# OnurBasci/TransformerBasedNavierStokeSolver

Measured on AMD Instinct MI355X. Metric: ns64_train_samples_per_s, higher is better.
Workload: dtype f32

## Files before the change

transformerbasednavierstokesolver_amd/csrc/pa2d_gemm.hip:

```cpp
#include "pa2d_gemm_common.h"
#include <string.h>

static bool engine_ok(int e) { return e >= 0 && e <= 2; }

static Pa2dEnv read_env() {
    auto is = [](const char* n, const char* pre) { const char* e = getenv(n); return e && strncmp(e, pre, strlen(pre)) == 0; };
    auto num = [](const char* n, int dflt) { const char* e = getenv(n); return (e && e[0]) ? atoi(e) : dflt; };
    Pa2dEnv v;
    v.conv_halo = is("PA2D_CONV_HALO", "o") ? 0 : (is("PA2D_CONV_HALO", "f") ? 2 : 1);
    v.mc_big_off = is("PA2D_MC_BIG", "o") ? 1 : 0;
    v.kc_bk16 = num("PA2D_KC_BK", 0) == 16 ? 1 : 0;
    v.mc_bk = num("PA2D_MC_BK", 16) == 32 ? 32 : 16;
    v.mc_splits = num("PA2D_MC_SPLITS", 0);
    v.mcb_splits = num("PA2D_MCB_SPLITS", 0);
    v.lin_dw_split = is("PA2D_LIN_DW_SPLIT", "of") ? 0 : 1;
    v.lin_panel = is("PA2D_LIN_PANEL", "of") ? 0 : 1;
    v.lin_rowpanel = is("PA2D_LIN_ROWPANEL", "of") ? 0 : 1;
    v.lin_small_split = is("PA2D_LIN_SMALL_SPLIT", "of") ? 0 : 1;
    v.conv_mfma16 = num("PA2D_CONV_MFMA", 16) == 32 ? 0 : 1;
    v.split_big = num("PA2D_SPLIT_BIG", 1);
    v.slice_map = is("PA2D_SLICE_MAP", "l") ? 0 : 1;
    v.default_engine = is("PA2D_GEMM", "f") ? 0 : (is("PA2D_GEMM", "b") ? 2 : 1);
    return v;
}
static Pa2dEnv g_env = read_env();
const Pa2dEnv& pa2d_env() { return g_env; }
static int kc_bk(bool im2col, int Cin) {
    if (im2col && pa2d_env().kc_bk16) return 16;
    return (!im2col || (Cin % 32) == 0) ? 32 : 16;
}
KCTile kc_tile(int M, int N, bool im2col, int Cin) {
    const int tiles_m = ceil_div(M, 128);
    const long long t128 = (long long)tiles_m * ceil_div(N, 128);
    const long long t12864 = (long long)tiles_m * ceil_div(N, 64);
    const int bk = kc_bk(im2col, Cin);
    if (N > 64 && t128 >= 384) return {128, 128, bk};
    if (t12864 >= 384 || M <= 64) return {128, 64, bk};
    return {64, 64, bk};
}
bool use_split(int engine, int N, bool im2col, int Cin) {
    const int m = engine;
    if (m == 1) return im2col && N > 64 && (Cin % 32) == 0;
    if (m == 2) return N > 64 && (!im2col || (Cin % 32) == 0);
    return false;
}

static int launch_kc(const KCParams& p_in, bool im2col, hipStream_t st, hipEvent_t ev0 = nullptr, hipEvent_t ev1 = nullptr);
static int launch_kc(const KCParams& p_in, bool im2col, hipStream_t st, hipEvent_t ev0, hipEvent_t ev1) {
    KCParams p = p_in;
    if (!engine_ok(p.engine)) return PA2D_ERR_ARG;
    if (p.M <= 0 || p.N <= 0 || p.K <= 0) return PA2D_OK;
    if (!p.bias2) p.bias_split = 0x7fffffff;
    {
        const unsigned long long ab = ((unsigned long long)(p.M - 1) * p.lda + (im2col ? p.Cin : p.K)) * 4ull;
        const unsigned long long bb = ((unsigned long long)(p.N - 1) * p.ldb + p.K) * 4ull;
        if (ab >= 0xFFFFFFF0ull || bb >= 0xFFFFFFF0ull) return PA2D_ERR_UNSUPPORTED;
        p.a_bytes = (unsigned)ab;
        p.b_bytes = (unsigned)bb;
        const unsigned long long es = p.io_bf16 ? 2ull : 4ull;
        const unsigned long long cb = ((unsigned long long)(p.M - 1) * p.ldc + p.N) * es;
        const unsigned long long rb = p.res ? ((unsigned long long)(p.M - 1) * p.ldres + p.N) * es : 0ull;
        const unsigned long long xb = p.aux ? ((unsigned long long)(p.M - 1) * p.ldaux + p.N) * es : 0ull;
        if (cb >= 0xFFFFFFF0ull || rb >= 0xFFFFFFF0ull || xb >= 0xFFFFFFF0ull) return PA2D_ERR_UNSUPPORTED;
        p.c_bytes = (unsigned)cb; p.res_bytes = (unsigned)rb; p.aux_bytes = (unsigned)xb;
    }
    if ((p.K & 3) || (p.lda & 3) || (p.ldb & 3)) return PA2D_ERR_ARG;
    if (im2col && ((p.Cin & 15) || p.K != 9 * p.Cin)) return PA2D_ERR_UNSUPPORTED;
    if (im2col && (p.epi != 0 || p.res)) return PA2D_ERR_ARG;
    if (ev0 && hipEventRecord(ev0, st) != hipSuccess) return PA2D_ERR_ARG;
    int rc;
    if (!im2col && p.wimg && rowpanel_applies(p)) {
        if (p.wsrc) {
            rc = launch_pack_weight_image(p.wsrc, p.wsn, p.wsk, p.wimg, p.N, p.K, st);
            if (rc) return rc;
        }
        KCParams pp = p;
        pp.M = p.M - p.M % 128;
        rc = launch_kc_rowpanel(pp, p.wimg, st);
        if (!rc && pp.M < p.M) {
            KCParams pt = p_in;
            pt.wimg = nullptr;
            pt.M = p.M - pp.M;
            pt.A = p.A + (size_t)pp.M * p.lda;
            pt.C = p.C + (size_t)pp.M * p.ldc;
            if (p.res) pt.res = p.res + (size_t)pp.M * p.ldres;
            if (p.aux) pt.aux = p.aux + (size_t)pp.M * p.ldaux;
            rc = launch_kc(pt, false, st);
        }
    } else if (panel_applies(p, im2col)) {
        KCParams pp = p;
        pp.M = p.M - p.M % 256;
        rc = launch_kc_panel(pp, st);
        if (!rc && pp.M < p.M) {
            KCParams pt = p_in;
            const size_t ea = p.io_bf16 ? 2 : 4, es = p.io_bf16 ? 2 : 4;
            pt.M = p.M - pp.M;
            pt.A = (const float*)((const char*)p.A + (size_t)pp.M * p.lda * ea);
            pt.C = (float*)((char*)p.C + (size_t)pp.M * p.ldc * es);
            if (p.res) pt.res = (const float*)((const char*)p.res + (size_t)pp.M * p.ldres * es);
            if (p.aux) pt.aux = (float*)((char*)p.aux + (size_t)pp.M * p.ldaux * es);
            rc = launch_kc(pt, false, st);
        }
    } else if (p.io_bf16 || use_split(p.engine, p.N, im2col, p.Cin)) rc = launch_kc_split(p, im2col, st);
    else if (kc_split_small_applies(p, im2col)) rc = launch_kc_split_small(p, st);
    else rc = launch_kc_f32(p, im2col, kc_tile(p.M, p.N, im2col, p.Cin), st);
    if (rc) return rc;
    if (ev1 && hipEventRecord(ev1, st) != hipSuccess) return PA2D_ERR_ARG;
    return PA2D_OK;
}

__global__ void repack_kernel(const float* __restrict__ w0, const float* __restrict__ w1, float* __restrict__ dst,
                              int mode, int N, int K, int C, int Cin) {
    const long long idx = (long long)blockIdx.x * blockDim.x + threadIdx.x;
    if (mode == 0) {
        if (idx >= (long long)N * K) return;
        const int n = (int)(idx % N), k = (int)(idx / N);
        dst[idx] = w0[(size_t)n * K + k];
    } else if (mode == 1) {
        if (idx >= (long long)2 * C * 9 * Cin) return;
        const int CH = K;
        const int c16 = (int)(idx % CH);
        const int tap = (int)((idx / CH) % 9);
        const int cic = (int)((idx / (9 * CH)) % (Cin / CH));
        const int co = (int)(idx / ((long long)Cin * 9));
        const int ci = cic * CH + c16;
        const float* src = co < C ? w0 : w1;
        dst[idx] = src[((size_t)(co % C) * Cin + ci) * 9 + tap];
    } else {
        if (idx >= (long long)2 * C * 9 * Cin) return;
        const int CH = K;
        const int c16 = (int)(idx % CH);
        const int tap = (int)((idx / CH) % 9);
        const int cic = (int)((idx / (9 * CH)) % (2 * C / CH));
        const int ci = (int)(idx / ((long long)2 * C * 9));
        const int co = cic * CH + c16;
        const float* src = co < C ? w0 : w1;
        dst[idx] = src[((size_t)(co % C) * Cin + ci) * 9 + (8 - tap)];
    }
}

static int launch_repack(const float* w0, const float* w1, float* dst, int mode, int N, int K, int C, int Cin,
                         hipStream_t st) {
    const long long count = mode == 0 ? (long long)N * K : (long long)2 * C * 9 * Cin;
    hipLaunchKernelGGL(repack_kernel, dim3((unsigned)ceil_div_ll(count, 256)), dim3(256), 0, st, w0, w1, dst, mode,
                       N, K, C, Cin);
    PA2D_CHECK_LAUNCH();
    return PA2D_OK;
}

extern "C" {

int pa2d_default_engine(void) { return pa2d_env().default_engine; }

void pa2d_reload_env(void) { g_env = read_env(); }

size_t pa2d_gemm_fwd_workspace(int N, int K, int engine) { return rowpanel_image_bytes(N, K, engine); }
size_t pa2d_gemm_bwd_data_workspace(int N, int K, int engine) {
    return (size_t)N * K * sizeof(float) + rowpanel_image_bytes(K, N, engine);
}

int pa2d_gemm_weight_image(const float* w, long long ldw, int transposed, void* img, size_t img_bytes, int N, int K,
                           int engine, hipStream_t st) {
    const size_t need = rowpanel_image_bytes(N, K, engine);
    if (need == 0) return PA2D_ERR_UNSUPPORTED;
    if (!img || img_bytes < need) return PA2D_ERR_WORKSPACE;
    return transposed ? launch_pack_weight_image(w, 1, ldw, img, N, K, st) : launch_pack_weight_image(w, ldw, 1, img, N, K, st);
}

int pa2d_gemm_bias_act_fwd(const float* x, long long ldx, const float* w, long long ldw, const float* bias,
                           const float* res, long long ldres, float* y, long long ldy, float* pre, long long ldpre,
                           const void* wimg, void* ws, size_t ws_bytes, int M, int N, int K, int act, int engine,
                           hipStream_t st) {
    KCParams p = {};
    p.engine = engine;
    p.aux_deriv = (act & PA2D_ACT_SAVE_DERIVATIVE_BIT) ? 1 : 0;
    act &= ~PA2D_ACT_SAVE_DERIVATIVE_BIT;
    p.A = x; p.lda = ldx; p.B = w; p.ldb = ldw; p.C = y; p.ldc = ldy; p.bias = bias; p.res = res; p.ldres = ldres;
    p.aux = pre; p.ldaux = ldpre; p.M = M; p.N = N; p.K = K; p.act = act;
    p.epi = (act != ACT_NONE ? EPI_ACT : 0) | (pre ? EPI_STORE_PRE : 0);
    const size_t img = rowpanel_image_bytes(N, K, engine);
    if (img && wimg) p.wimg = const_cast<void*>(wimg);
    else if (ws && img && ws_bytes >= img) { p.wimg = ws; p.wsrc = w; p.wsn = ldw; p.wsk = 1; }
    return launch_kc(p, false, st);
}

int pa2d_gemm_bwd_data(const float* dy, long long lddy, const float* w, long long ldw, const float* pre,
                       long long ldpre, int act, float* dx, long long lddx, const void* wimg, void* ws, size_t ws_bytes, int M,
                       int N, int K, int engine, hipStream_t st) {
    if (ldw != K) return PA2D_ERR_ARG;
    if (N & 3) return PA2D_ERR_ARG;
    if (M <= 0) return PA2D_OK;
    if (ws_bytes < (size_t)N * K * sizeof(float)) return PA2D_ERR_WORKSPACE;
    float* const wt_ws = (float*)ws;
    KCParams p = {};
    p.engine = engine;
    p.aux_deriv = (act & PA2D_ACT_SAVE_DERIVATIVE_BIT) ? 1 : 0;
    act &= ~PA2D_ACT_SAVE_DERIVATIVE_BIT;
    p.A = dy; p.lda = lddy; p.B = wt_ws; p.ldb = N; p.C = dx; p.ldc = lddx; p.M = M; p.N = K; p.K = N;
    p.aux = const_cast<float*>(pre); p.ldaux = ldpre; p.act = act;
    p.epi = (pre && act != ACT_NONE) ? EPI_MUL_DACT : 0;
    const size_t img = rowpanel_image_bytes(K, N, engine);
    if (img && wimg) p.wimg = const_cast<void*>(wimg);
    else if (img && ws_bytes >= (size_t)N * K * sizeof(float) + img) {
        p.wimg = (char*)ws + (size_t)N * K * sizeof(float); p.wsrc = w; p.wsn = 1; p.wsk = ldw;
    }
    if (!(p.wimg && rowpanel_applies(p) && (M % 128) == 0)) {
        const int rc = launch_repack(w, nullptr, wt_ws, 0, N, K, 0, 0, st);
        if (rc) return rc;
    }
    return launch_kc(p, false, st);
}

size_t pa2d_gemm_bwd_weight_workspace(int M, int N, int K, int engine) {
    (void)engine;
    const MCPlan pl = plan_mc(N, K, M);
    return (pl.slab_floats + (size_t)pl.splits * N) * sizeof(float);
}

int pa2d_gemm_bwd_weight(const float* dy, long long lddy, const float* x, long long ldx, float* dw, float* db,
                         void* ws, size_t ws_bytes, int M, int N, int K, int accumulate, int engine, hipStream_t st) {
    if (!engine_ok(engine)) return PA2D_ERR_ARG;
    if (M <= 0) {
        if (accumulate) return PA2D_OK;
        const int rz = pa2d_zero(dw, sizeof(float) * N * K, st);
        return rz ? rz : pa2d_zero(db, sizeof(float) * N, st);
    }
    if (ws_bytes < pa2d_gemm_bwd_weight_workspace(M, N, K, engine)) return PA2D_ERR_WORKSPACE;
    const MCPlan pl = plan_mc(N, K, M);
    float* cs = db ? (float*)ws + pl.slab_floats : nullptr;
    const bool bfk = (engine == 1 || engine == 2) && pl.big && mc_f32src_applies(N, K, M, lddy, ldx);
    int rc = bfk ? launch_mc_f32src(dy, lddy, N, x, ldx, K, M, (float*)ws, pl, engine == 2 ? 1 : 3, cs, st)
                 : launch_mc(dy, lddy, N, x, ldx, K, M, false, 0, 0, 0, (float*)ws, pl, engine, st, cs);
    if (rc) return rc;
    rc = launch_reduce((const float*)ws, pl.splits, (long long)N * K, dw, nullptr, 0, 0, 0, st, accumulate);
    if (rc) return rc;
    if (db) rc = launch_reduce(cs, pl.splits, N, db, nullptr, 0, 0, 0, st, accumulate);
    return rc;
}

static size_t conv_planes_bytes(int engine, int M, int N, int Cin) {
    if (!use_split(engine, N, true, Cin)) return 0;
    return (planes_bytes(M, Cin, engine == 2 ? 1 : 3) + 255) & ~(size_t)255;
}

static int conv_dw_kind(int engine, int M, int C) {
    if (conv_planes_bytes(engine, M, C, 2 * C) == 0) return 0;
    if (mc_planes_big_applies(C, C, M)) return 2;
    return (mc_planes_supported(C, C) && plan_mc(2 * C, 9 * C, M).big) ? 1 : 0;
}
static MCPlan conv_dw_plan(int engine, int M, int C) {
    return conv_dw_kind(engine, M, C) == 2 ? plan_mc_planes_big(2 * C, 9 * C, M) : plan_mc(2 * C, 9 * C, M);
}
static size_t conv_xplanes_bytes(int engine, int M, int C) {
    return conv_dw_kind(engine, M, C) ? ((planes_bytes(M, C, engine == 2 ? 1 : 3) + 255) & ~(size_t)255) : 0;
}

size_t pa2d_conv3x3x2_workspace(int B, int H, int W, int C, int engine) {
    const size_t pack = (size_t)3 * C * 9 * C;
    const MCPlan pl = conv_dw_plan(engine, B * H * W, C);
    size_t sl = pl.slab_floats, cs = (size_t)colsum_blocks(B * H * W) * 2 * C;
    return (pack + (sl > cs ? sl : cs)) * sizeof(float) + conv_planes_bytes(engine, B * H * W, C, 2 * C) +
           conv_xplanes_bytes(engine, B * H * W, C);
}

size_t pa2d_conv3x3x2_fwd_workspace(int B, int H, int W, int C, int engine) {
    return (size_t)3 * C * 9 * C * sizeof(float) + conv_planes_bytes(engine, B * H * W, 2 * C, C);
}

static int conv_pack(const float* wx, const float* wf, float* pack, int M, int C, int direction, int engine,
                     hipStream_t st) {
    const int N = direction ? C : 2 * C, Cin = direction ? 2 * C : C;
    if (use_split(engine, N, true, Cin)) {
        return launch_repack_split(wx, wf, pack, direction, engine == 2 ? 1 : 3, C, C, st);
    }
    return launch_repack(wx, wf, pack, direction ? 2 : 1, 0, kc_tile(M, N, true, Cin).bk, C, C, st);
}

size_t pa2d_conv3x3x2_pack_bytes(int C) { return (size_t)3 * C * 9 * C * sizeof(float); }

int pa2d_conv3x3x2_pack(const float* wx, const float* wf, void* pack, size_t pack_bytes, int B, int H, int W, int C,
                        int direction, int engine, hipStream_t st) {
    if (!engine_ok(engine)) return PA2D_ERR_ARG;
    if (pack_bytes < pa2d_conv3x3x2_pack_bytes(C)) return PA2D_ERR_WORKSPACE;
    return conv_pack(wx, wf, (float*)pack, B * H * W, C, direction ? 1 : 0, engine, st);
}

int pa2d_conv3x3x2_fwd(const float* xn, const float* wx, const float* bx, const float* wf, const float* bf,
                       float* out, const void* prepacked, void* ws, size_t ws_bytes, int B, int H, int W, int C,
                       int engine, hipStream_t st, hipEvent_t ev_start, hipEvent_t ev_stop) {
    if (!engine_ok(engine)) return PA2D_ERR_ARG;
    if (B <= 0) return PA2D_OK;
    if (ws_bytes < pa2d_conv3x3x2_fwd_workspace(B, H, W, C, engine)) return PA2D_ERR_WORKSPACE;
    const float* pack = (const float*)prepacked;
    if (!pack) {
        const int rc = conv_pack(wx, wf, (float*)ws, B * H * W, C, 0, engine, st);
        if (rc) return rc;
        pack = (const float*)ws;
    }
    const size_t apl = conv_planes_bytes(engine, B * H * W, 2 * C, C);
    void* const planes = (char*)ws + pa2d_conv3x3x2_pack_bytes(C);
    if (apl) {
        const int rc = launch_split_planes(xn, C, planes, (long long)B * H * W, C, engine == 2 ? 1 : 3, st);
        if (rc) return rc;
    }
    KCParams p = {};
    p.engine = engine;
    p.A = apl ? (const float*)planes : xn; p.apre = apl ? 1 : 0;
    p.lda = C; p.B = pack; p.ldb = 9 * C; p.C = out; p.ldc = 2 * C;
    p.bias = bx; p.bias2 = bf; p.bias_split = C;
    p.M = B * H * W; p.N = 2 * C; p.K = 9 * C; p.H = H; p.W = W; p.Cin = C;
    return launch_kc(p, true, st, ev_start, ev_stop);
}

int pa2d_conv3x3x2_bwd(const float* dout, const float* xn, const float* wx, const float* wf, float* dxn, float* dwx,
                       float* dbx, float* dwf, float* dbf, const void* prepacked, void* ws, size_t ws_bytes, int B,
                       int H, int W, int C, int accumulate, int engine, hipStream_t st, hipEvent_t ev_start,
                       hipEvent_t ev_stop) {
    if (!engine_ok(engine)) return PA2D_ERR_ARG;
    if (B <= 0) {
        if (accumulate) return PA2D_OK;
        const size_t wb = sizeof(float) * (size_t)C * C * 9, bb = sizeof(float) * C;
        int rz = pa2d_zero(dwx, wb, st);
// ... 259 lines not shown
```

transformerbasednavierstokesolver_amd/csrc/pa2d_gemm_mc_planes.hip:

```cpp
#include "pa2d_gemm_common.h"

typedef short s16x4 __attribute__((ext_vector_type(4)));
typedef short s16x8 __attribute__((ext_vector_type(8)));

struct MCPlanesParams {
    const void* PA; int chA;
    const void* PB; int chB;
    float* slab;
    int Mi, Nj, Mk, chunks_per_split, splits, H, W, Cin;
    unsigned a_bytes, b_bytes;
    int taps;
    long long lda, ldb;
    float* colsum;
};

__device__ __forceinline__ unsigned img_off(int row, int ch) {
    return 256u * row + 16u * (ch ^ (((row & 3) << 2) | ((row >> 2) & 3)));
}

template <int NT, int KS, bool F32SRC = false>
__global__ __launch_bounds__(256, 2) void gemm_mc_planes_kernel(const MCPlanesParams p) {
    constexpr int PIMG = 4096;
    constexpr int STAGE = 2 * NT * KS * PIMG;
    constexpr int NP = 2 * NT * KS;
// ... 80 lines not shown
            rg[s] = s_isb[s] ? __builtin_amdgcn_raw_buffer_load_b128(rb_rsrc, ok_ ? rowb_ + s_goff[s] : OOB_OFF, 0, 0) \
                             : __builtin_amdgcn_raw_buffer_load_b128(ra_rsrc, ok_ ? rowb_ + s_goff[s] : OOB_OFF, 0, 0); \
        }                                                                                                 \
    }
#define MP_STORE(buf_)                                                                                    \
    if constexpr (F32SRC) {                                                                               \
        _Pragma("unroll") for (int ks = 0; ks < KS; ++ks) _Pragma("unroll") for (int op = 0; op < 2; ++op) { \
            const u32x4 u0_ = rg[ks * 4 + op * 2], u1_ = rg[ks * 4 + op * 2 + 1];                         \
            const float4 v0_ = make_float4(__uint_as_float(u0_.x), __uint_as_float(u0_.y), __uint_as_float(u0_.z), __uint_as_float(u0_.w)); \
            const float4 v1_ = make_float4(__uint_as_float(u1_.x), __uint_as_float(u1_.y), __uint_as_float(u1_.z), __uint_as_float(u1_.w)); \
            if (op == 0 && do_cs) {                                                                       \
                cs[0] += v0_.x; cs[1] += v0_.y; cs[2] += v0_.z; cs[3] += v0_.w;                           \
                cs[4] += v1_.x; cs[5] += v1_.y; cs[6] += v1_.z; cs[7] += v1_.w;                           \
            }                                                                                             \
            bf16x4 h0_, m0_, l0_, h1_, m1_, l1_;                                                          \
            split3(v0_, h0_, m0_, l0_);                                                                   \
            split3(v1_, h1_, m1_, l1_);                                                                   \
            unsigned char* d_ = smem + (buf_) * STAGE + flds;                                             \
            *reinterpret_cast<bf16x8*>(d_ + ((op * NT + 0) * KS + ks) * PIMG) = __builtin_shufflevector(h0_, h1_, 0, 1, 2, 3, 4, 5, 6, 7); \
            if (NT == 3) {                                                                                \
                *reinterpret_cast<bf16x8*>(d_ + ((op * NT + 1) * KS + ks) * PIMG) = __builtin_shufflevector(m0_, m1_, 0, 1, 2, 3, 4, 5, 6, 7); \
                *reinterpret_cast<bf16x8*>(d_ + ((op * NT + 2) * KS + ks) * PIMG) = __builtin_shufflevector(l0_, l1_, 0, 1, 2, 3, 4, 5, 6, 7); \
            }                                                                                             \
        }                                                                                                 \
    } else {                                                                                              \
        _Pragma("unroll") for (int s = 0; s < NP; ++s)                                                    \
            *reinterpret_cast<u32x4*>(smem + (buf_) * STAGE + s_lds[s]) = rg[s];                          \
    }
    const bool do_cs = F32SRC && p.colsum != nullptr && tj == 0;

    f32x16 acc[2][2];
#pragma unroll
    for (int i = 0; i < 2; ++i)
#pragma unroll
        for (int j = 0; j < 2; ++j)
#pragma unroll
            for (int r = 0; r < 16; ++r) acc[i][j][r] = 0.f;

    const int g = lane >> 4, q4 = (lane & 15) >> 2, pq = lane & 3;
    unsigned fa[2][2], fb[2][2];
#pragma unroll
    for (int t = 0; t < 2; ++t)
#pragma unroll
        for (int r = 0; r < 2; ++r) {
            const int row = 8 * (g >> 1) + 4 * r + q4;
            const int cha = ((wm * 64 + t * 32) >> 3) + 2 * (g & 1) + (pq >> 1);
            const int chb = ((wn * 64 + t * 32) >> 3) + 2 * (g & 1) + (pq >> 1);
            fa[t][r] = img_off(row, cha) + 8u * (pq & 1);
            fb[t][r] = img_off(row, chb) + 8u * (pq & 1);
        }

    if (c_begin < c_end) {
        MP_LOAD(c_begin)
        MP_STORE(0)
    }
    __syncthreads();
    for (int c = c_begin; c < c_end; c += KS) {
        const int buf = ((c - c_begin) / KS) & 1;
        if (c + KS < c_end) { MP_LOAD(c + KS) }
#pragma unroll
        for (int ks = 0; ks < KS; ++ks) {
        const unsigned char* st = smem + buf * STAGE + ks * PIMG;
        bf16x8 af[2][NT], bf[2][NT];
#pragma unroll
        for (int t = 0; t < 2; ++t)
#pragma unroll
            for (int pl = 0; pl < NT; ++pl) {
                typedef __attribute__((address_space(3))) s16x4 lds_s16x4;
                const s16x4 a0 = __builtin_amdgcn_ds_read_tr16_b64_v4i16((lds_s16x4*)(st + pl * KS * PIMG + fa[t][0]));
                const s16x4 a1 = __builtin_amdgcn_ds_read_tr16_b64_v4i16((lds_s16x4*)(st + pl * KS * PIMG + fa[t][1]));
                const s16x4 b0 = __builtin_amdgcn_ds_read_tr16_b64_v4i16((lds_s16x4*)(st + (NT + pl) * KS * PIMG + fb[t][0]));
                const s16x4 b1 = __builtin_amdgcn_ds_read_tr16_b64_v4i16((lds_s16x4*)(st + (NT + pl) * KS * PIMG + fb[t][1]));
                const s16x8 av = __builtin_shufflevector(a0, a1, 0, 1, 2, 3, 4, 5, 6, 7);
                const s16x8 bv = __builtin_shufflevector(b0, b1, 0, 1, 2, 3, 4, 5, 6, 7);
                af[t][pl] = __builtin_bit_cast(bf16x8, av);
                bf[t][pl] = __builtin_bit_cast(bf16x8, bv);
            }
#pragma unroll
        for (int i = 0; i < 2; ++i)
#pragma unroll
            for (int j = 0; j < 2; ++j) {
                if constexpr (NT == 3) {
                    acc[i][j] = __builtin_amdgcn_mfma_f32_32x32x16_bf16(af[i][1], bf[j][1], acc[i][j], 0, 0, 0);
                    acc[i][j] = __builtin_amdgcn_mfma_f32_32x32x16_bf16(af[i][2], bf[j][0], acc[i][j], 0, 0, 0);
                    acc[i][j] = __builtin_amdgcn_mfma_f32_32x32x16_bf16(af[i][0], bf[j][2], acc[i][j], 0, 0, 0);
                    acc[i][j] = __builtin_amdgcn_mfma_f32_32x32x16_bf16(af[i][1], bf[j][0], acc[i][j], 0, 0, 0);
                    acc[i][j] = __builtin_amdgcn_mfma_f32_32x32x16_bf16(af[i][0], bf[j][1], acc[i][j], 0, 0, 0);
                }
                acc[i][j] = __builtin_amdgcn_mfma_f32_32x32x16_bf16(af[i][0], bf[j][0], acc[i][j], 0, 0, 0);
            }
        }
        if (c + KS < c_end) { MP_STORE(buf ^ 1) }
        __syncthreads();
    }
#undef MP_LOAD
#undef MP_STORE

    if constexpr (F32SRC) {
        if (do_cs) {
            float* sm = reinterpret_cast<float*>(smem);
#pragma unroll
            for (int e = 0; e < 8; ++e) sm[frow * 128 + fc8 * 8 + e] = cs[e];
            __syncthreads();
            if (tid < 128) {
                float t = 0.f;
#pragma unroll
                for (int r = 0; r < 16; ++r) t += sm[r * 128 + tid];
                if (ti * 128 + tid < p.Mi) p.colsum[(size_t)split * p.Mi + ti * 128 + tid] = t;
            }
        }
    }
    float* out = p.slab + (size_t)split * p.Mi * p.Nj;
    const int col0 = tj * 128 + wn * 64 + (lane & 31);
    const int row0 = ti * 128 + wm * 64 + 4 * (lane >> 5);
#pragma unroll
    for (int j = 0; j < 2; ++j)
#pragma unroll
        for (int i = 0; i < 2; ++i)
#pragma unroll
            for (int r = 0; r < 16; ++r) {
                const int row = row0 + i * 32 + (r & 3) + 8 * (r >> 2);
                if (!F32SRC || (row < p.Mi && col0 + j * 32 < p.Nj)) out[(size_t)row * p.Nj + col0 + j * 32] = acc[i][j][r];
            }
}

bool mc_planes_supported(int C, int Cin) { return (C % 64) == 0 && (Cin % 128) == 0; }

int launch_mc_planes(const void* PA, const void* PB, int C, int Cin, int Mk, int H, int W, float* slab,
                     const MCPlan& pl, int NT, hipStream_t st) {
    if (!mc_planes_supported(C, Cin) || !pl.big) return PA2D_ERR_UNSUPPORTED;
    MCPlanesParams p;
    p.PA = PA; p.chA = 2 * C / 32; p.PB = PB; p.chB = Cin / 32; p.slab = slab;
    p.Mi = 2 * C; p.Nj = 9 * Cin; p.Mk = Mk; p.chunks_per_split = pl.chunks_per_split; p.splits = pl.splits;
    p.H = H; p.W = W; p.Cin = Cin; p.taps = 9;
    const unsigned long long ab = (unsigned long long)Mk * p.chA * NT * 64, bb = (unsigned long long)Mk * p.chB * NT * 64;
    if (ab >= 0xFFFFFFF0ull || bb >= 0xFFFFFFF0ull) return PA2D_ERR_UNSUPPORTED;
    p.a_bytes = (unsigned)ab; p.b_bytes = (unsigned)bb;
    const dim3 grid((p.Mi / 128) * (p.Nj / 128) * pl.splits);
    if (NT == 3) hipLaunchKernelGGL((gemm_mc_planes_kernel<3, 1>), grid, dim3(256), 0, st, p);
    else hipLaunchKernelGGL((gemm_mc_planes_kernel<1, 4>), grid, dim3(256), 0, st, p);
    PA2D_CHECK_LAUNCH();
    return PA2D_OK;
}

template <int NT, int KS>
__global__ __launch_bounds__(512, 1) void gemm_mc_planes_big_kernel(const MCPlanesParams p, const int per_xcd) {
    constexpr int PIMG = 8192;
    constexpr int STAGE = 2 * NT * KS * PIMG;
    constexpr int NP = (2 * NT * KS * 512) / 512;
    extern __shared__ __attribute__((aligned(16))) unsigned char smem[];

    const int tid = threadIdx.x, lane = tid & 63, wave = tid >> 6;
    const int tiles_i = (p.Mi + 255) / 256, tiles_j = (p.Nj + 255) / 256;
    const int tiles = tiles_i * tiles_j;
    const int lin = (blockIdx.x & 7) * per_xcd + (blockIdx.x >> 3);
    if ((int)(blockIdx.x >> 3) >= per_xcd || lin >= tiles * p.splits) return;
    const int split = lin / tiles, t_ = lin - split * tiles;
    const int ti = t_ / tiles_j, tj = t_ - ti * tiles_j;
    const int wm = wave >> 2, wn = wave & 3;
    const int total_chunks = (p.Mk + 15) / 16;
    const int c_begin = split * p.chunks_per_split;
    const int c_end = min(total_chunks, c_begin + p.chunks_per_split);
    const int HW = p.taps == 1 ? 1 : p.H * p.W;

    const __amdgpu_buffer_rsrc_t ra_rsrc = __builtin_amdgcn_make_buffer_rsrc(const_cast<void*>(p.PA), 0, p.a_bytes, 0x00020000);
    const __amdgpu_buffer_rsrc_t rb_rsrc = __builtin_amdgcn_make_buffer_rsrc(const_cast<void*>(p.PB), 0, p.b_bytes, 0x00020000);

    const int row16 = tid >> 5, cgrp = (tid & 31) >> 2, piece = tid & 3;
    const bool colok_a = ti * 256 + cgrp * 32 < p.Mi;
    const unsigned goff_a = (unsigned)((((ti * 256) >> 5) + cgrp) * NT * 64 + piece * 16);
    const int jc = tj * 256 + cgrp * 32;
    const int tap = p.taps == 1 ? 4 : jc / p.Cin;
    const bool colok_b = jc < p.Nj;
    const unsigned goff_b = (unsigned)((p.taps == 1 ? (jc >> 5) : ((jc - tap * p.Cin) >> 5)) * NT * 64 + piece * 16);
    const int tap_dy = tap / 3 - 1, tap_dx = tap - (tap / 3) * 3 - 1, tap_shift = tap_dy * p.W + tap_dx;
    const unsigned pitch_a = (unsigned)(p.chA * NT * 64), pitch_b = (unsigned)(p.chB * NT * 64);
    const unsigned lds_off = 512u * row16 + 16u * ((unsigned)(cgrp * 4 + piece) ^ (unsigned)(((row16 & 3) << 2) | ((row16 >> 2) & 3)));
#define MB_LOAD(c_, RG)                                                                                   \
    {                                                                                                     \
        _Pragma("unroll") for (int ks = 0; ks < KS; ++ks) {                                               \
            const int m_ = ((c_) + ks) * 16 + row16;                                                      \
            const bool okr_ = m_ < p.Mk && (c_) + ks < c_end;             \
            bool okb_ = okr_ && colok_b;                                                                  \
            int mm_ = m_;                                                                                 \
            if (p.taps != 1) {       \
                okb_ = okb_ && (unsigned)(ly + tap_dy) < (unsigned)p.H && (unsigned)(lx + tap_dx) < (unsigned)p.W; \
                mm_ = m_ + tap_shift;                                                                     \
                lx += 16;                                                                                 \
                while (lx >= p.W) { lx -= p.W; ++ly; }                                                    \
                while (ly >= p.H) ly -= p.H;                                                              \
            }                                                                                             \
            const unsigned oa_ = (okr_ && colok_a) ? (unsigned)m_ * pitch_a + goff_a : OOB_OFF;           \
            const unsigned ob_ = okb_ ? (unsigned)mm_ * pitch_b + goff_b : OOB_OFF;                       \
            _Pragma("unroll") for (int pl = 0; pl < NT; ++pl) {                                           \
                RG[pl * KS + ks] = __builtin_amdgcn_raw_buffer_load_b128(ra_rsrc, oa_ == OOB_OFF ? OOB_OFF : oa_ + pl * 64u, 0, 0); \
                RG[(NT + pl) * KS + ks] = __builtin_amdgcn_raw_buffer_load_b128(rb_rsrc, ob_ == OOB_OFF ? OOB_OFF : ob_ + pl * 64u, 0, 0); \
            }                                                                                             \
        }                                                                                                 \
    }
#define MB_STORE(buf_, RG)                                                                                \
    {                                                                                                     \
        _Pragma("unroll") for (int s = 0; s < NP; ++s)                                                    \
            *reinterpret_cast<u32x4*>(smem + (buf_) * STAGE + s * PIMG + lds_off) = RG[s];                \
    }
    u32x4 rg0[NP];
    int ly = 0, lx = 0;
    if (p.taps != 1) {
        const int n0 = (c_begin * 16 + row16) % HW;
        ly = n0 / p.W;
        lx = n0 - ly * p.W;
    }

    f32x16 acc[4][2];
#pragma unroll
    for (int i = 0; i < 4; ++i)
#pragma unroll
        for (int j = 0; j < 2; ++j)
#pragma unroll
            for (int r = 0; r < 16; ++r) acc[i][j][r] = 0.f;

    const int g = lane >> 4, q4 = (lane & 15) >> 2, pq = lane & 3;
    unsigned fa[4][2], fb[2][2];
#pragma unroll
    for (int r = 0; r < 2; ++r) {
        const int row = 8 * (g >> 1) + 4 * r + q4;
        const unsigned swz = (unsigned)(((row & 3) << 2) | ((row >> 2) & 3));
#pragma unroll
        for (int t = 0; t < 4; ++t) {
            const int cha = ((wm * 128 + t * 32) >> 3) + 2 * (g & 1) + (pq >> 1);
            fa[t][r] = 512u * row + 16u * ((unsigned)cha ^ swz) + 8u * (pq & 1);
        }
#pragma unroll
        for (int t = 0; t < 2; ++t) {
            const int chb = ((wn * 64 + t * 32) >> 3) + 2 * (g & 1) + (pq >> 1);
            fb[t][r] = 512u * row + 16u * ((unsigned)chb ^ swz) + 8u * (pq & 1);
        }
    }

#define MB_COMPUTE(buf_)                                                                                  \
    _Pragma("unroll") for (int ks = 0; ks < KS; ++ks) {                                                   \
        const unsigned char* st = smem + (buf_) * STAGE + ks * PIMG;                                      \
        bf16x8 af[4][NT], bf[2][NT];                                                                      \
        typedef __attribute__((address_space(3))) s16x4 lds_s16x4;                                        \
        _Pragma("unroll") for (int pl = 0; pl < NT; ++pl) {                                               \
            _Pragma("unroll") for (int t = 0; t < 4; ++t) {                                               \
                const s16x4 a0 = __builtin_amdgcn_ds_read_tr16_b64_v4i16((lds_s16x4*)(st + pl * KS * PIMG + fa[t][0])); \
                const s16x4 a1 = __builtin_amdgcn_ds_read_tr16_b64_v4i16((lds_s16x4*)(st + pl * KS * PIMG + fa[t][1])); \
                af[t][pl] = __builtin_bit_cast(bf16x8, __builtin_shufflevector(a0, a1, 0, 1, 2, 3, 4, 5, 6, 7)); \
            }                                                                                             \
            _Pragma("unroll") for (int t = 0; t < 2; ++t) {                                               \
                const s16x4 b0 = __builtin_amdgcn_ds_read_tr16_b64_v4i16((lds_s16x4*)(st + (NT + pl) * KS * PIMG + fb[t][0])); \
                const s16x4 b1 = __builtin_amdgcn_ds_read_tr16_b64_v4i16((lds_s16x4*)(st + (NT + pl) * KS * PIMG + fb[t][1])); \
                bf[t][pl] = __builtin_bit_cast(bf16x8, __builtin_shufflevector(b0, b1, 0, 1, 2, 3, 4, 5, 6, 7)); \
            }                                                                                             \
        }                                                                                                 \
        _Pragma("unroll") for (int i = 0; i < 4; ++i)                                                     \
            _Pragma("unroll") for (int j = 0; j < 2; ++j) {                                               \
                if constexpr (NT == 3) {                                        \
                    acc[i][j] = __builtin_amdgcn_mfma_f32_32x32x16_bf16(af[i][1], bf[j][1], acc[i][j], 0, 0, 0); \
                    acc[i][j] = __builtin_amdgcn_mfma_f32_32x32x16_bf16(af[i][2], bf[j][0], acc[i][j], 0, 0, 0); \
                    acc[i][j] = __builtin_amdgcn_mfma_f32_32x32x16_bf16(af[i][0], bf[j][2], acc[i][j], 0, 0, 0); \
                    acc[i][j] = __builtin_amdgcn_mfma_f32_32x32x16_bf16(af[i][1], bf[j][0], acc[i][j], 0, 0, 0); \
                    acc[i][j] = __builtin_amdgcn_mfma_f32_32x32x16_bf16(af[i][0], bf[j][1], acc[i][j], 0, 0, 0); \
                }                                                                                         \
                acc[i][j] = __builtin_amdgcn_mfma_f32_32x32x16_bf16(af[i][0], bf[j][0], acc[i][j], 0, 0, 0); \
            }                                                                                             \
    }
    if (c_begin < c_end) {
        MB_LOAD(c_begin, rg0)
        MB_STORE(0, rg0)
        if (c_begin + KS < c_end) MB_LOAD(c_begin + KS, rg0)
    }
    __syncthreads();
    for (int c = c_begin; c < c_end; c += KS) {
        const int buf = ((c - c_begin) / KS) & 1;
        if (c + KS < c_end) {
            MB_STORE(buf ^ 1, rg0)
            if (c + 2 * KS < c_end) MB_LOAD(c + 2 * KS, rg0)
        }
        MB_COMPUTE(buf)
        __syncthreads();
    }
#undef MB_COMPUTE
#undef MB_LOAD
#undef MB_STORE

    float* out = p.slab + (size_t)split * p.Mi * p.Nj;
    const int col0 = tj * 256 + wn * 64 + (lane & 31);
    const int row0 = ti * 256 + wm * 128 + 4 * (lane >> 5);
#pragma unroll
    for (int j = 0; j < 2; ++j) {
        const int col = col0 + j * 32;
        if (col >= p.Nj) continue;
#pragma unroll
        for (int i = 0; i < 4; ++i)
#pragma unroll
            for (int r = 0; r < 16; ++r) {
                const int row = row0 + i * 32 + (r & 3) + 8 * (r >> 2);
                if (row < p.Mi) out[(size_t)row * p.Nj + col] = acc[i][j][r];
            }
    }
}

MCPlan plan_mc_planes_big(int Mi, int Nj, int Mk) {
    MCPlan pl;
    if (Mk < 1) Mk = 1;
    pl.big = 2;
    const int tiles = ceil_div(Mi, 256) * ceil_div(Nj, 256);
    const int total_chunks = ceil_div(Mk, 16);
    int splits = 256 / tiles;
    if (pa2d_env().mcb_splits > 0) splits = pa2d_env().mcb_splits;
    const int max_splits = total_chunks / 8 > 0 ? total_chunks / 8 : 1;
    if (splits > max_splits) splits = max_splits;
    if (splits < 1) splits = 1;
    pl.chunks_per_split = ceil_div(total_chunks, splits);
    pl.splits = ceil_div(total_chunks, pl.chunks_per_split);
    pl.slab_floats = (size_t)pl.splits * Mi * Nj;
    return pl;
}

bool mc_planes_big_applies(int C, int Cin, int Mk) {
    if (pa2d_env().mc_big_off) return false;
    return (C % 16) == 0 && (Cin % 32) == 0 && 2 * C >= 256 && 9 * Cin >= 256 && Mk >= 16 * 8 * 4;
}

int launch_mc_planes_big(const void* PA, const void* PB, int C, int Cin, int Mk, int H, int W, float* slab,
                         const MCPlan& pl, int NT, hipStream_t st) {
    return launch_mc_planes_big_raw(PA, 2 * C, PB, Cin, 9, Mk, H, W, slab, pl, NT, st);
}

int launch_mc_planes_big_raw(const void* PA, int Mi, const void* PB, int Cin, int taps, int Mk, int H, int W, float* slab,
                             const MCPlan& pl, int NT, hipStream_t st) {
    if ((Mi & 31) || (Cin & 31) || (taps != 1 && taps != 9)) return PA2D_ERR_UNSUPPORTED;
    MCPlanesParams p;
    p.PA = PA; p.chA = Mi / 32; p.PB = PB; p.chB = Cin / 32; p.slab = slab;
    p.Mi = Mi; p.Nj = taps * Cin; p.Mk = Mk; p.chunks_per_split = pl.chunks_per_split; p.splits = pl.splits;
    p.H = H; p.W = W; p.Cin = Cin; p.taps = taps;
    const unsigned long long ab = (unsigned long long)Mk * p.chA * NT * 64, bb = (unsigned long long)Mk * p.chB * NT * 64;
    if (ab >= 0xFFFFFFF0ull || bb >= 0xFFFFFFF0ull) return PA2D_ERR_UNSUPPORTED;
    p.a_bytes = (unsigned)ab; p.b_bytes = (unsigned)bb;
    const int wgs = ceil_div(p.Mi, 256) * ceil_div(p.Nj, 256) * pl.splits;
    const int per_xcd = ceil_div(wgs, 8);
    const dim3 grid(per_xcd * 8);
    if (NT == 3) {
        const int smem = 2 * 2 * 3 * 1 * 8192;
        {
            hipError_t e = hipFuncSetAttribute(reinterpret_cast<const void*>(&gemm_mc_planes_big_kernel<3, 1>),
                                               hipFuncAttributeMaxDynamicSharedMemorySize, smem);
            if (e != hipSuccess) return (int)e;
        }
        hipLaunchKernelGGL((gemm_mc_planes_big_kernel<3, 1>), grid, dim3(512), smem, st, p, per_xcd);
    } else {
        const int smem = 2 * 2 * 1 * 4 * 8192;
        {
            hipError_t e = hipFuncSetAttribute(reinterpret_cast<const void*>(&gemm_mc_planes_big_kernel<1, 4>),
                                               hipFuncAttributeMaxDynamicSharedMemorySize, smem);
            if (e != hipSuccess) return (int)e;
        }
        hipLaunchKernelGGL((gemm_mc_planes_big_kernel<1, 4>), grid, dim3(512), smem, st, p, per_xcd);
    }
    PA2D_CHECK_LAUNCH();
    return PA2D_OK;
}

bool mc_f32src_applies(int Mi, int Nj, int Mk, long long lda, long long ldb) {
    return pa2d_env().lin_dw_split && (Mi % 8) == 0 && (Nj % 8) == 0 && Mi > 64 && Nj > 64 && Mk >= 16 * 8 * 16 && (lda % 4) == 0 && (ldb % 4) == 0;
}

int launch_mc_f32src(const float* A, long long lda, int Mi, const float* B, long long ldb, int Nj, int Mk, float* slab,
                     const MCPlan& pl, int NT, float* colsum, hipStream_t st) {
    if (!pl.big) return PA2D_ERR_UNSUPPORTED;
    MCPlanesParams p = {};
    p.PA = A; p.PB = B; p.slab = slab; p.lda = lda; p.ldb = ldb; p.colsum = colsum;
    p.Mi = Mi; p.Nj = Nj; p.Mk = Mk; p.chunks_per_split = pl.chunks_per_split; p.splits = pl.splits;
    p.H = 1; p.W = 1; p.Cin = Nj; p.taps = 1; p.chA = 0; p.chB = 0;
    const unsigned long long ab = ((unsigned long long)(Mk - 1) * lda + Mi) * 4ull, bb = ((unsigned long long)(Mk - 1) * ldb + Nj) * 4ull;
    if (ab >= 0xFFFFFFF0ull || bb >= 0xFFFFFFF0ull) return PA2D_ERR_UNSUPPORTED;
    p.a_bytes = (unsigned)ab; p.b_bytes = (unsigned)bb;
    const dim3 grid(ceil_div(Mi, 128) * ceil_div(Nj, 128) * pl.splits);
    if (NT == 3) hipLaunchKernelGGL((gemm_mc_planes_kernel<3, 1, true>), grid, dim3(256), 0, st, p);
    else hipLaunchKernelGGL((gemm_mc_planes_kernel<1, 4, true>), grid, dim3(256), 0, st, p);
    PA2D_CHECK_LAUNCH();
    return PA2D_OK;
}
```

transformerbasednavierstokesolver_amd/csrc/pa2d_internal.h:

```cpp
#pragma once
#include <hip/hip_runtime.h>
#include <stdint.h>

typedef float f32x16 __attribute__((ext_vector_type(16)));
typedef float f32x4 __attribute__((ext_vector_type(4)));

#define PA2D_OK 0
#define PA2D_ERR_ARG 1001
#define PA2D_ERR_UNSUPPORTED 1002
#define PA2D_ERR_WORKSPACE 1003

#define PA2D_CHECK_LAUNCH()                         \
    do {                                            \
        hipError_t e__ = hipGetLastError();         \
        if (e__ != hipSuccess) return (int)e__;     \
    } while (0)

enum { ACT_NONE = 0, ACT_GELU = 1, ACT_TANH = 2, ACT_SIGMOID = 3, ACT_RELU = 4, ACT_SOFTPLUS = 5,
       ACT_ELU = 6, ACT_SILU = 7 };

__device__ __forceinline__ float normal_cdf(float x, float& e_out) {
#pragma clang fp contract(off)
    const float z = fabsf(x) * 0.70710678118654752440f;
    const float t = __builtin_amdgcn_rcpf(fmaf(0.3275911f, z, 1.0f));
    float poly = fmaf(1.061405429f, t, -1.453152027f);
    poly = fmaf(poly, t, 1.421413741f);
    poly = fmaf(poly, t, -0.284496736f);
    poly = fmaf(poly, t, 0.254829592f);
    const float e = __builtin_amdgcn_exp2f(-z * z * 1.44269504088896340736f);
    e_out = e;
    const float hq = 0.5f * poly * t * e;
    return x < 0.f ? hq : 1.0f - hq;
}
__device__ __forceinline__ float gelu_exact(float x) {
#pragma clang fp contract(off)
    float e;
    return x * normal_cdf(x, e);
}
__device__ __forceinline__ float dgelu_exact(float x) {
#pragma clang fp contract(off)
    float e;
    const float cdf = normal_cdf(x, e);
    return fmaf(x * 0.39894228040143267794f, e, cdf);
}

__device__ __forceinline__ float act_fwd(int id, float x) {
    switch (id) {
        case ACT_GELU: return gelu_exact(x);
        case ACT_TANH: return tanhf(x);
        case ACT_SIGMOID: return 1.0f / (1.0f + expf(-x));
        case ACT_RELU: return x > 0.f ? x : 0.f;
        case ACT_SOFTPLUS: return x > 20.f ? x : log1pf(expf(x));
        case ACT_ELU: return x > 0.f ? x : expm1f(x);
        case ACT_SILU: return x / (1.0f + expf(-x));
        default: return x;
    }
}

__device__ __forceinline__ float act_bwd(int id, float x) {
    switch (id) {
        case ACT_GELU: return dgelu_exact(x);
        case ACT_TANH: { const float t = tanhf(x); return 1.0f - t * t; }
        case ACT_SIGMOID: { const float s = 1.0f / (1.0f + expf(-x)); return s * (1.0f - s); }
        case ACT_RELU: return x > 0.f ? 1.f : 0.f;
        case ACT_SOFTPLUS: return x > 20.f ? 1.f : 1.0f / (1.0f + expf(-x));
        case ACT_ELU: return x > 0.f ? 1.f : expf(x);
        case ACT_SILU: { const float s = 1.0f / (1.0f + expf(-x)); return s * (1.0f + x * (1.0f - s)); }
        default: return 1.f;
    }
}

__device__ __forceinline__ float wave_sum(float v) {
#pragma unroll
    for (int o = 32; o > 0; o >>= 1) v += __shfl_xor(v, o, 64);
    return v;
}
__device__ __forceinline__ float wave_max(float v) {
#pragma unroll
    for (int o = 32; o > 0; o >>= 1) v = fmaxf(v, __shfl_xor(v, o, 64));
    return v;
}

typedef unsigned int u32x4 __attribute__((ext_vector_type(4)));
#define OOB_OFF 0xFFFFFFFFu

__device__ __forceinline__ __amdgpu_buffer_rsrc_t make_rsrc(const float* base, unsigned bytes) {
    return __builtin_amdgcn_make_buffer_rsrc(const_cast<float*>(base), 0, bytes, 0x00020000);
}
__device__ __forceinline__ float4 buf_load4(__amdgpu_buffer_rsrc_t r, unsigned voff) {
    const u32x4 v = __builtin_amdgcn_raw_buffer_load_b128(r, voff, 0, 0);
    return make_float4(__uint_as_float(v.x), __uint_as_float(v.y), __uint_as_float(v.z), __uint_as_float(v.w));
}


__device__ __forceinline__ float buf_load1(__amdgpu_buffer_rsrc_t r, unsigned voff) {
    return __uint_as_float(__builtin_amdgcn_raw_buffer_load_b32(r, voff, 0, 0));
}
__device__ __forceinline__ void buf_store1(__amdgpu_buffer_rsrc_t r, unsigned voff, float v) {
    __builtin_amdgcn_raw_buffer_store_b32(__float_as_uint(v), r, voff, 0, 0);
}

__device__ __forceinline__ float2 buf_load2(__amdgpu_buffer_rsrc_t r, unsigned voff) {
    typedef unsigned int u32x2_ __attribute__((ext_vector_type(2)));
    const u32x2_ v = __builtin_amdgcn_raw_buffer_load_b64(r, voff, 0, 0);
    return make_float2(__uint_as_float(v.x), __uint_as_float(v.y));
}
__device__ __forceinline__ void buf_store4(__amdgpu_buffer_rsrc_t r, unsigned voff, float4 v) {
    u32x4 u = {__float_as_uint(v.x), __float_as_uint(v.y), __float_as_uint(v.z), __float_as_uint(v.w)};
    __builtin_amdgcn_raw_buffer_store_b128(u, r, voff, 0, 0);
}

#define PA2D_ACT_SAVE_DERIVATIVE_BIT 0x100

struct Pa2dEnv {
    int conv_halo;
    int mc_big_off;
    int kc_bk16;
    int mc_bk;
    int mc_splits;
    int mcb_splits;
    int lin_dw_split;
    int lin_panel;
    int conv_mfma16;
    int lin_small_split;
    int lin_rowpanel;
    int split_big;
    int slice_map;
    int default_engine;
};
const Pa2dEnv& pa2d_env();

static inline int pa2d_zero(void* p, size_t bytes, hipStream_t st) {
    if (!p || !bytes) return PA2D_OK;
    return (int)hipMemsetAsync(p, 0, bytes, st);
}
static inline int ceil_div(int a, int b) { return (a + b - 1) / b; }
static inline long long ceil_div_ll(long long a, long long b) { return (a + b - 1) / b; }

struct ReduceSegs { int nseg; long long begin[5]; float* dst[4]; };
int pa2d_launch_reduce_segs(const float* slab, int nslab, long long count, const ReduceSegs& segs, int accumulate,
                            hipStream_t st);

typedef __bf16 bf16_t;
template <typename T> struct Act;
template <> struct Act<float> {
    static constexpr unsigned ES = 4;
    static __device__ __forceinline__ float4 ld4(const float* p) { return *reinterpret_cast<const float4*>(p); }
    static __device__ __forceinline__ void st4(float* p, float4 v) { *reinterpret_cast<float4*>(p) = v; }
    static __device__ __forceinline__ float ld1(const float* p) { return *p; }
    static __device__ __forceinline__ float4 bld4(__amdgpu_buffer_rsrc_t r, unsigned off) { return buf_load4(r, off); }
    static __device__ __forceinline__ float2 bld2(__amdgpu_buffer_rsrc_t r, unsigned off) { return buf_load2(r, off); }
    static __device__ __forceinline__ float bld1(__amdgpu_buffer_rsrc_t r, unsigned off) { return buf_load1(r, off); }
    static __device__ __forceinline__ float bld1s(__amdgpu_buffer_rsrc_t r, unsigned off, unsigned soff) {
        return __uint_as_float(__builtin_amdgcn_raw_buffer_load_b32(r, off, soff, 0));
    }
    static __device__ __forceinline__ void bst4(__amdgpu_buffer_rsrc_t r, unsigned off, float4 v) { buf_store4(r, off, v); }
    static __device__ __forceinline__ void bst1(__amdgpu_buffer_rsrc_t r, unsigned off, float v) { buf_store1(r, off, v); }
};
__device__ __forceinline__ float bf16_bits_to_f32(unsigned short b) { return __uint_as_float((unsigned)b << 16); }
__device__ __forceinline__ unsigned short f32_to_bf16_bits(float x) {
    const bf16_t h = (bf16_t)x;
    return __builtin_bit_cast(unsigned short, h);
}
__device__ __forceinline__ unsigned pack_bf16x2(float lo, float hi) {
    return (unsigned)f32_to_bf16_bits(lo) | ((unsigned)f32_to_bf16_bits(hi) << 16);
}
template <> struct Act<bf16_t> {
    static constexpr unsigned ES = 2;
    static __device__ __forceinline__ float4 unpack4(uint2 q) {
        return make_float4(__uint_as_float(q.x << 16), __uint_as_float(q.x & 0xFFFF0000u), __uint_as_float(q.y << 16),
                           __uint_as_float(q.y & 0xFFFF0000u));
    }
    static __device__ __forceinline__ float4 ld4(const bf16_t* p) { return unpack4(*reinterpret_cast<const uint2*>(p)); }
    static __device__ __forceinline__ void st4(bf16_t* p, float4 v) {
        *reinterpret_cast<uint2*>(p) = make_uint2(pack_bf16x2(v.x, v.y), pack_bf16x2(v.z, v.w));
    }
    static __device__ __forceinline__ float ld1(const bf16_t* p) { return (float)*p; }
    static __device__ __forceinline__ float4 bld4(__amdgpu_buffer_rsrc_t r, unsigned off) {
        typedef unsigned int u32x2_ __attribute__((ext_vector_type(2)));
        const u32x2_ q = __builtin_amdgcn_raw_buffer_load_b64(r, off, 0, 0);
        return unpack4(make_uint2(q.x, q.y));
    }
    static __device__ __forceinline__ float2 bld2(__amdgpu_buffer_rsrc_t r, unsigned off) {
        const unsigned q = __builtin_amdgcn_raw_buffer_load_b32(r, off, 0, 0);
        return make_float2(__uint_as_float(q << 16), __uint_as_float(q & 0xFFFF0000u));
    }
    static __device__ __forceinline__ float bld1(__amdgpu_buffer_rsrc_t r, unsigned off) {
        return bf16_bits_to_f32(__builtin_amdgcn_raw_buffer_load_b16(r, off, 0, 0));
    }
    static __device__ __forceinline__ float bld1s(__amdgpu_buffer_rsrc_t r, unsigned off, unsigned soff) {
        return bf16_bits_to_f32(__builtin_amdgcn_raw_buffer_load_b16(r, off, soff, 0));
    }
    static __device__ __forceinline__ void bst4(__amdgpu_buffer_rsrc_t r, unsigned off, float4 v) {
        typedef unsigned int u32x2_ __attribute__((ext_vector_type(2)));
        const u32x2_ q = {pack_bf16x2(v.x, v.y), pack_bf16x2(v.z, v.w)};
        __builtin_amdgcn_raw_buffer_store_b64(q, r, off, 0, 0);
    }
    static __device__ __forceinline__ void bst1(__amdgpu_buffer_rsrc_t r, unsigned off, float v) {
        __builtin_amdgcn_raw_buffer_store_b16(f32_to_bf16_bits(v), r, off, 0, 0);
    }
};
__device__ __forceinline__ __amdgpu_buffer_rsrc_t make_rsrc_v(const void* base, unsigned bytes) {
    return __builtin_amdgcn_make_buffer_rsrc(const_cast<void*>(base), 0, bytes, 0x00020000);
}

__device__ __forceinline__ bool slice_decode(int xcd_map, int B, int heads, int nchunk, int& b, int& hh, int& chunk, int& bid) {
    const int total = B * heads * nchunk;
    int L;
    if (xcd_map) {
        const int per = (total + 7) >> 3;
        if ((int)(blockIdx.x >> 3) >= per) return false;
        L = (int)(blockIdx.x & 7) * per + (int)(blockIdx.x >> 3);
        if (L >= total) return false;
        hh = L % heads;
        chunk = (L / heads) % nchunk;
        b = L / (heads * nchunk);
    } else {
        L = (int)blockIdx.x;
        if (L >= total) return false;
        chunk = L % nchunk;
        hh = (L / nchunk) % heads;
        b = L / (nchunk * heads);
    }
    bid = (b * heads + hh) * nchunk + chunk;
    return true;
}
static inline int slice_grid(int total) { return ((total + 7) / 8) * 8; }
```

Measured before the change: 68.13.

## Add 16x16x32 MFMA variant of big wgrad planes GEMM kernel

Adds a new 3-plane (NT=3) weight-gradient GEMM kernel that uses 16x16x32 bf16 MFMA with transposed LDS reads, instead of the 32x32 MFMA path. It uses a three-slot LDS ring and splits each K-chunk's compute into two halves so the next loads overlap with the MFMAs. It is the default, selectable through PA2D_WGRAD_MFMA. The aim is better MFMA throughput and latency hiding for the big wgrad GEMMs, at the cost of more LDS per block (launch bounds 512,1) and more code.

```diff
diff --git a/transformerbasednavierstokesolver_amd/csrc/pa2d_gemm.hip b/transformerbasednavierstokesolver_amd/csrc/pa2d_gemm.hip
--- a/transformerbasednavierstokesolver_amd/csrc/pa2d_gemm.hip
+++ b/transformerbasednavierstokesolver_amd/csrc/pa2d_gemm.hip
@@ -18,6 +18,7 @@
     v.lin_rowpanel = is("PA2D_LIN_ROWPANEL", "of") ? 0 : 1;
     v.lin_small_split = is("PA2D_LIN_SMALL_SPLIT", "of") ? 0 : 1;
     v.conv_mfma16 = num("PA2D_CONV_MFMA", 16) == 32 ? 0 : 1;
+    v.wgrad_mfma16 = num("PA2D_WGRAD_MFMA", 16) == 32 ? 0 : 1;
     v.split_big = num("PA2D_SPLIT_BIG", 1);
     v.slice_map = is("PA2D_SLICE_MAP", "l") ? 0 : 1;
     v.default_engine = is("PA2D_GEMM", "f") ? 0 : (is("PA2D_GEMM", "b") ? 2 : 1);
diff --git a/transformerbasednavierstokesolver_amd/csrc/pa2d_gemm_mc_planes.hip b/transformerbasednavierstokesolver_amd/csrc/pa2d_gemm_mc_planes.hip
--- a/transformerbasednavierstokesolver_amd/csrc/pa2d_gemm_mc_planes.hip
+++ b/transformerbasednavierstokesolver_amd/csrc/pa2d_gemm_mc_planes.hip
@@ -406,6 +406,167 @@
     }
 }
 
+template <int NT>
+__global__ __launch_bounds__(512, 1) void gemm_mc_planes_big16_kernel(const MCPlanesParams p, const int per_xcd) {
+    constexpr int PIMG = 8192;
+    constexpr int UNIT = 2 * NT * PIMG;
+    constexpr int NP = 2 * NT;
+    extern __shared__ __attribute__((aligned(16))) unsigned char smem[];
+
+    const int tid = threadIdx.x, lane = tid & 63, wave = tid >> 6;
+    const int tiles_i = (p.Mi + 255) / 256, tiles_j = (p.Nj + 255) / 256;
+    const int tiles = tiles_i * tiles_j;
+    const int lin = (blockIdx.x & 7) * per_xcd + (blockIdx.x >> 3);
+    if ((int)(blockIdx.x >> 3) >= per_xcd || lin >= tiles * p.splits) return;
+    const int split = lin / tiles, t_ = lin - split * tiles;
+    const int ti = t_ / tiles_j, tj = t_ - ti * tiles_j;
+    const int wm = wave >> 2, wn = wave & 3;
+    const int total_chunks = (p.Mk + 15) / 16;
+    const int c_begin = split * p.chunks_per_split;
+    const int c_end = min(total_chunks, c_begin + p.chunks_per_split);
+    const int HW = p.taps == 1 ? 1 : p.H * p.W;
+
+    const __amdgpu_buffer_rsrc_t ra_rsrc = __builtin_amdgcn_make_buffer_rsrc(const_cast<void*>(p.PA), 0, p.a_bytes, 0x00020000);
+    const __amdgpu_buffer_rsrc_t rb_rsrc = __builtin_amdgcn_make_buffer_rsrc(const_cast<void*>(p.PB), 0, p.b_bytes, 0x00020000);
+
+    const int row16 = tid >> 5, cgrp = (tid & 31) >> 2, piece = tid & 3;
+    const bool colok_a = ti * 256 + cgrp * 32 < p.Mi;
+    const unsigned goff_a = (unsigned)((((ti * 256) >> 5) + cgrp) * NT * 64 + piece * 16);
+    const int jc = tj * 256 + cgrp * 32;
+    const int tap = p.taps == 1 ? 4 : jc / p.Cin;
+    const bool colok_b = jc < p.Nj;
+    const unsigned goff_b = (unsigned)((p.taps == 1 ? (jc >> 5) : ((jc - tap * p.Cin) >> 5)) * NT * 64 + piece * 16);
+    const int tap_dy = tap / 3 - 1, tap_dx = tap - (tap / 3) * 3 - 1, tap_shift = tap_dy * p.W + tap_dx;
+    const unsigned pitch_a = (unsigned)(p.chA * NT * 64), pitch_b = (unsigned)(p.chB * NT * 64);
+    const unsigned lds_off = 512u * row16 + 16u * ((unsigned)(cgrp * 4 + piece) ^ (unsigned)(((row16 & 3) << 2) | ((row16 >> 2) & 3)));
+    int ly = 0, lx = 0;
+    if (p.taps != 1) {
+        const int n0 = (c_begin * 16 + row16) % HW;
+        ly = n0 / p.W;
+        lx = n0 - ly * p.W;
+    }
+#define MB16_LOAD(c_)                                                                                     \
+    {                                                                                                     \
+        const int m_ = (c_) * 16 + row16;                                                                 \
+        const bool okr_ = m_ < p.Mk && (c_) < c_end;                                                      \
+        bool okb_ = okr_ && colok_b;                                                                      \
+        int mm_ = m_;                                                                                     \
+        if (p.taps != 1) {                                                                                \
+            okb_ = okb_ && (unsigned)(ly + tap_dy) < (unsigned)p.H && (unsigned)(lx + tap_dx) < (unsigned)p.W; \
+            mm_ = m_ + tap_shift;                                                                         \
+            lx += 16;                                                                                     \
+            while (lx >= p.W) { lx -= p.W; ++ly; }                                                        \
+            while (ly >= p.H) ly -= p.H;                                                                  \
+        }                                                                                                 \
+        const unsigned oa_ = (okr_ && colok_a) ? (unsigned)m_ * pitch_a + goff_a : OOB_OFF;               \
+        const unsigned ob_ = okb_ ? (unsigned)mm_ * pitch_b + goff_b : OOB_OFF;                           \
+        _Pragma("unroll") for (int pl = 0; pl < NT; ++pl) {                                               \
+            rg[pl] = __builtin_amdgcn_raw_buffer_load_b128(ra_rsrc, oa_ == OOB_OFF ? OOB_OFF : oa_ + pl * 64u, 0, 0); \
+            rg[NT + pl] = __builtin_amdgcn_raw_buffer_load_b128(rb_rsrc, ob_ == OOB_OFF ? OOB_OFF : ob_ + pl * 64u, 0, 0); \
+        }                                                                                                 \
+    }
+#define MB16_STORE(slot_)                                                                                 \
+    {                                                                                                     \
+        _Pragma("unroll") for (int s = 0; s < NP; ++s)                                                    \
+            *reinterpret_cast<u32x4*>(smem + (slot_) * UNIT + s * PIMG + lds_off) = rg[s];                \
+    }
+    u32x4 rg[NP];
+
+    f32x4 acc[8][4];
+#pragma unroll
+    for (int i = 0; i < 8; ++i)
+#pragma unroll
+        for (int j = 0; j < 4; ++j) acc[i][j] = f32x4{0.f, 0.f, 0.f, 0.f};
+
+    const int g = lane >> 4, q4 = (lane & 15) >> 2, pq = lane & 3, second = g >> 1;
+    unsigned fa[2], fb[2];
+#pragma unroll
+    for (int r = 0; r < 2; ++r) {
+        const int row = 8 * (g & 1) + 4 * r + q4;
+        const unsigned swz = (unsigned)(((row & 3) << 2) | ((row >> 2) & 3));
+        fa[r] = 512u * row + 16u * ((unsigned)(wm * 16 + (pq >> 1)) ^ swz) + 8u * (pq & 1);
+        fb[r] = 512u * row + 16u * ((unsigned)(wn * 8 + (pq >> 1)) ^ swz) + 8u * (pq & 1);
+    }
+    typedef __attribute__((address_space(3))) s16x4 lds_s16x4;
+#define MB16_FRAG(base_, off0_, off1_, t_)                                                                \
+    __builtin_bit_cast(bf16x8, __builtin_shufflevector(                                                  \
+        __builtin_amdgcn_ds_read_tr16_b64_v4i16((lds_s16x4*)((base_) + ((off0_) ^ (32u * (t_))))),        \
+        __builtin_amdgcn_ds_read_tr16_b64_v4i16((lds_s16x4*)((base_) + ((off1_) ^ (32u * (t_))))), 0, 1, 2, 3, 4, 5, 6, 7))
+#define MB16_COMPUTE(i0_)                                                                                 \
+    {                                                                                                     \
+        bf16x8 af[2][NT];                                                                                 \
+        _Pragma("unroll") for (int pl = 0; pl < NT; ++pl) af[0][pl] = MB16_FRAG(st + pl * PIMG, fa[0], fa[1], (i0_)); \
+        _Pragma("unroll") for (int i = (i0_); i < (i0_) + 4; ++i) {                                       \
+            const int cur = (i - (i0_)) & 1;                                                              \
+            if (i + 1 < (i0_) + 4)                                                                        \
+                _Pragma("unroll") for (int pl = 0; pl < NT; ++pl) af[cur ^ 1][pl] = MB16_FRAG(st + pl * PIMG, fa[0], fa[1], i + 1); \
+            _Pragma("unroll") for (int j = 0; j < 4; ++j) {                                               \
+                if constexpr (NT == 3) {                                        \
+                    acc[i][j] = __builtin_amdgcn_mfma_f32_16x16x32_bf16(af[cur][1], bf[j][1], acc[i][j], 0, 0, 0); \
+                    acc[i][j] = __builtin_amdgcn_mfma_f32_16x16x32_bf16(af[cur][2], bf[j][0], acc[i][j], 0, 0, 0); \
+                    acc[i][j] = __builtin_amdgcn_mfma_f32_16x16x32_bf16(af[cur][0], bf[j][2], acc[i][j], 0, 0, 0); \
+                    acc[i][j] = __builtin_amdgcn_mfma_f32_16x16x32_bf16(af[cur][1], bf[j][0], acc[i][j], 0, 0, 0); \
+                    acc[i][j] = __builtin_amdgcn_mfma_f32_16x16x32_bf16(af[cur][0], bf[j][1], acc[i][j], 0, 0, 0); \
+                }                                                                                         \
+                acc[i][j] = __builtin_amdgcn_mfma_f32_16x16x32_bf16(af[cur][0], bf[j][0], acc[i][j], 0, 0, 0); \
+            }                                                                                             \
+        }                                                                                                 \
+    }
+
+    int sA = 0, sB = 1, sF = 2;
+    if (c_begin < c_end) {
+        MB16_LOAD(c_begin)
+        MB16_STORE(0)
+        MB16_LOAD(c_begin + 1)
+        MB16_STORE(1)
+        if (c_begin + 2 < c_end) MB16_LOAD(c_begin + 2)
+    }
+    __syncthreads();
+    for (int c = c_begin; c < c_end; c += 2) {
+        const bool more = c + 2 < c_end;
+        if (c != c_begin && more) MB16_LOAD(c + 2)
+        const unsigned char* st = smem + (second ? sB : sA) * UNIT;
+        bf16x8 bf[4][NT];
+#pragma unroll
+        for (int pl = 0; pl < NT; ++pl)
+#pragma unroll
+            for (int j = 0; j < 4; ++j) bf[j][pl] = MB16_FRAG(st + (NT + pl) * PIMG, fb[0], fb[1], j);
+        MB16_COMPUTE(0)
+        if (more) {
+            MB16_STORE(sF)
+            MB16_LOAD(c + 3)
+        }
+        MB16_COMPUTE(4)
+        __syncthreads();
+        if (more) {
+            MB16_STORE(sA)
+            __syncthreads();
+        }
+        const int s0 = sA;
+        sA = sF; sF = sB; sB = s0;
+    }
+#undef MB16_COMPUTE
+#undef MB16_FRAG
+#undef MB16_LOAD
+#undef MB16_STORE
+
+    float* out = p.slab + (size_t)split * p.Mi * p.Nj;
+    const int col0 = tj * 256 + wn * 64 + (lane & 15);
+    const int row0 = ti * 256 + wm * 128 + 4 * (lane >> 4);
+#pragma unroll
+    for (int j = 0; j < 4; ++j) {
+        const int col = col0 + j * 16;
+        if (col >= p.Nj) continue;
+#pragma unroll
+        for (int i = 0; i < 8; ++i)
+#pragma unroll
+            for (int r = 0; r < 4; ++r) {
+                const int row = row0 + i * 16 + r;
+                if (row < p.Mi) out[(size_t)row * p.Nj + col] = acc[i][j][r];
+            }
+    }
+}
+
 MCPlan plan_mc_planes_big(int Mi, int Nj, int Mk) {
     MCPlan pl;
     if (Mk < 1) Mk = 1;
@@ -446,7 +607,15 @@
     const int wgs = ceil_div(p.Mi, 256) * ceil_div(p.Nj, 256) * pl.splits;
     const int per_xcd = ceil_div(wgs, 8);
     const dim3 grid(per_xcd * 8);
-    if (NT == 3) {
+    if (NT == 3 && pa2d_env().wgrad_mfma16) {
+        const int smem = 3 * 2 * 3 * 8192;
+        {
+            hipError_t e = hipFuncSetAttribute(reinterpret_cast<const void*>(&gemm_mc_planes_big16_kernel<3>),
+                                               hipFuncAttributeMaxDynamicSharedMemorySize, smem);
+            if (e != hipSuccess) return (int)e;
+        }
+        hipLaunchKernelGGL((gemm_mc_planes_big16_kernel<3>), grid, dim3(512), smem, st, p, per_xcd);
+    } else if (NT == 3) {
         const int smem = 2 * 2 * 3 * 1 * 8192;
         {
             hipError_t e = hipFuncSetAttribute(reinterpret_cast<const void*>(&gemm_mc_planes_big_kernel<3, 1>),
diff --git a/transformerbasednavierstokesolver_amd/csrc/pa2d_internal.h b/transformerbasednavierstokesolver_amd/csrc/pa2d_internal.h
--- a/transformerbasednavierstokesolver_amd/csrc/pa2d_internal.h
+++ b/transformerbasednavierstokesolver_amd/csrc/pa2d_internal.h
@@ -122,6 +122,7 @@
     int lin_dw_split;
     int lin_panel;
     int conv_mfma16;
+    int wgrad_mfma16;
     int lin_small_split;
     int lin_rowpanel;
     int split_big;
```

Result: faster. 69.25, median of 6 (+1.6%).
